# LorenzoNajt/FlipComplexityEmpirical

Measured on AMD Instinct MI355X. Metric: flip proposals/sec (node) 40x40 grid k=2, 1/2/4/8 MI355X; % LDS/HBM roofline, higher is better.
Workload: dtype int8

## Files before the change

flipcomplexityempirical_amd/csrc/fc_capi.cpp:

```cpp
#include <algorithm>
#include <cstdio>
#include <cstdlib>
#include <cstring>
#include <memory>
#include <new>
#include <string>
#include <vector>

#include "fc_run.h"

struct fc_graph {
    fc::HostGraph h;
};

namespace {

constexpr int kWaveSlots = 64;
thread_local std::string g_err;

}

int fc::fail(int code, const std::string &msg) {
    g_err = msg;
    return code;
// ... 228 lines not shown
    for (int32_t c = 0; c < r->n_chains; ++c) {
        fc::ChainScalars &s = sc[c];
        const int64_t w = fc::geom_from(fc::u53(words[2 * c], words[2 * c + 1]), r->log1mp[s.nb]);
        s.sum_wait += w - s.wait_cur;
        s.wait_cur = w;
    }
    HIP_TRY(hipMemcpy(r->d_sc, sc.data(), sc.size() * sizeof(sc[0]), hipMemcpyHostToDevice));
    return FC_OK;
}

#ifdef FC_PHASE_PROF
static int dump_prof(fc_run *r, hipStream_t s) {
    if (const char *path = std::getenv("FC_PROF_OUT")) {
        std::vector<int64_t> h((size_t)r->n_chains * fc::kProfSlots);
        HIP_TRY(hipStreamSynchronize(s));
        HIP_TRY(hipMemcpy(h.data(), r->d_prof, h.size() * 8, hipMemcpyDeviceToHost));
        if (FILE *f = std::fopen(path, "ab")) {
            std::fwrite(h.data(), 8, h.size(), f);
            std::fclose(f);
        }
    }
    return FC_OK;
}
#endif

static fc::KParams flip_params(const fc_run *r, int64_t n_steps, int64_t max_draws) {
    fc::KParams k{};
    k.graph = r->d_graph;
    k.ring_eid = r->d_ring_eid;
    k.n = r->g.n;
    k.n_edges = r->g.n_edges;
    k.n_chains = r->n_chains;
    k.k = r->p.k;
    k.popk = r->d_popk;
    k.all_exact = r->g.n_exact == r->g.n ? 1 : 0;
    k.dgraph = r->dgraph ? 1 : 0;
    k.mcnt = r->d_mcnt;
    k.ngk = r->d_ngk;
    k.wmax = r->wmax > 0 ? r->wmax : 1;
    k.wdyn = r->p.k > 2 && r->wmax <= 0 ? 1 : 0;
    k.nfh = r->d_nfh;
    k.band = r->d_sbits ? 1 : 0;
    k.sbits = r->d_sbits;
    k.band_step0 = 1;
    while (k.band_step0 * 2 < r->words) k.band_step0 *= 2;
    k.chain_lds_bytes = r->chain_lds_bytes;
    k.words = r->words;
    k.lab_words = fc::bfs_lab_words(r->g.n);
    k.lemire_thresh = (uint32_t)((1ull << 32) % (uint64_t)r->g.n);
    k.chain_id_offset = r->p.chain_id_offset;
    k.seed_lo = (uint32_t)r->p.seed;
    k.seed_hi = (uint32_t)(r->p.seed >> 32);
    k.pop_lo = (int32_t)r->p.pop_lo;
    k.n_steps = n_steps;
    k.max_draws = max_draws > 0 ? max_draws : 65536 * std::max<int64_t>(n_steps, 1);
    k.assign = r->d_assign;
    k.fcnt = r->d_fcnt;
    k.sc = r->d_sc;
    k.thresh = r->d_thresh;
    k.log1mp = r->d_log1mp;
    k.pkeys = r->d_pkeys;
    k.labels = r->d_labels;
    k.diag = r->p.diag_mask;
    k.flags = r->p.flags;
    k.cut_hist = r->d_cut_hist;
    k.nb_hist = r->d_nb_hist;
    k.nb_w = r->nb_w;
    k.nb_pairs = (r->p.flags & FC_FLAG_NB_PAIRS) && r->p.k > 2;
    k.edge_acc = r->d_edge_acc;
    k.num_flips = r->d_num_flips;
    k.part_sum = r->d_part_sum;
    k.last_flipped = r->d_last_flipped;
    k.flip_count = r->d_flip_count;
    k.occ_acc = r->d_occ_acc;
    k.last_accept = r->d_last_accept;
    k.trace = r->d_trace;
    k.trace_chains = r->p.trace_chains;
    k.trace_cap = r->p.trace_cap;
    k.tape = r->d_tape;
    k.tape_draws = r->tape_draws;
    k.events = r->d_events;
    k.ev_cap = r->ev_cap;
    k.hit_lo = r->p.hit_lo;
    k.hit_hi = r->p.hit_hi;
    k.nsub = r->tune.nsub;
    k.hit_stop = r->tune.hit_stop;
    k.par_min = r->tune.par_min;
    k.multi_flip = r->tune.multi ? r->mf_marks : 0;
    k.wait_q = r->tune.wait_q;
    k.wpb = r->tune.wpb;
    k.coop = r->tune.coop ? 1 : 0;
    k.variant = r->variant ? 1 : 0;
    k.accept = r->p.accept;
    k.con_valid = r->p.con_valid;
    k.con_accept = r->p.con_accept;
    if (r->variant) k.par_min = kWaveSlots + 1;
    for (int i = 0; i < 3; ++i) {
        k.prio_nb[i] = r->tune.prio_div[0] > 0 && r->p.k == 2 ? k.n / r->tune.prio_div[i] : 0;
        k.prio_th[i] = r->tune.prio_th[i];
    }
    return k;
}

static fc::RecomParams recom_params(const fc_run *r, int64_t n_steps, int64_t max_draws, int64_t *prof) {
    fc::RecomParams q{};
    q.graph = r->d_graph;
    q.nbe = r->d_nbe;
    q.eslot = r->d_eslot;
    q.nb_d = r->nb_d;
    q.eu = r->d_eu;
    q.ev = r->d_ev;
    q.n = r->g.n;
    q.n_edges = r->g.n_edges;
    q.n_chains = r->n_chains;
// ... 91 lines not shown
    HIP_TRY(hipSetDevice(r->p.device));
    fc::KParams k = flip_params(r, n_steps, max_draws);
    hipStream_t s = hip_stream ? (hipStream_t)hip_stream : r->stream;
#ifdef FC_PHASE_PROF
    if (!r->d_prof) {
        if (int rc = r->d_prof.alloc((size_t)r->n_chains * fc::kProfSlots)) return rc;
    }
    HIP_TRY(hipMemsetAsync(r->d_prof, 0, (size_t)r->n_chains * fc::kProfSlots * 8, s));
    k.prof = r->d_prof;
#endif
    size_t slot_i;
    if (int rc = take_event_slot(r, &slot_i)) return rc;
    const auto evp = r->launch_events[slot_i];
    HIP_TRY(hipEventRecord(evp.first, s));
    if (r->p.proposal == FC_PROPOSE_RECOM) {
        const fc::RecomParams q = recom_params(r, n_steps, max_draws, k.prof);
        const int e = fc::launch_recom(q, r->g.ring_max, s, r->kname, sizeof r->kname);
        if (e != 0) return fail(FC_ERR_HIP, std::string("recom kernel launch: ") + hipGetErrorString((hipError_t)e));
        return finish_launches(r, evp, s);
    }
    constexpr int64_t kChunk = int64_t(1) << 24;
    if (r->p.k == 2 && k.prio_nb[0] > 0 && k.prio_th[0] >= 0.0f) {
        if (!r->d_eta) {
            if (int rc = r->d_eta.alloc(2)) return rc;
            HIP_TRY(hipMemsetAsync(r->d_eta, 0, 2 * sizeof(uint32_t), s));
        }
        k.eta = r->d_eta;
    }
    if (r->tune.deal) {
        if (!r->d_deal) {
            if (int rc = r->d_deal.alloc((size_t)fc::kDealKeys + 4)) return rc;
            if (int rc = r->d_order.alloc((size_t)r->n_chains)) return rc;
            if (int rc = r->d_ctime.alloc((size_t)r->n_chains)) return rc;
        }
        k.deal = r->d_deal;
        k.order = r->d_order;
        k.ctime = r->d_ctime;
    }
    int64_t chunk = kChunk;
    if (int rc = size_tally_log(r, n_steps, s, k, &chunk)) return rc;
    for (int64_t done = 0; done < n_steps; done += chunk) {
        k.n_steps = std::min(chunk, n_steps - done);
        if (max_draws <= 0) k.max_draws = 65536 * k.n_steps;
        if (k.order) {
            const int e = fc::launch_deal_order(r->d_ctime, r->d_sc, k.n, r->n_chains, r->deal_timed ? 1 : 0,
                                                r->d_order, r->d_deal, s);
            if (e != 0) return fail(FC_ERR_HIP, std::string("deal kernel launch: ") + hipGetErrorString((hipError_t)e));
            r->deal_timed = true;
        }
        if (k.eta) {
            k.eta_parity = (int32_t)(r->n_flip_launches++ & 1);
            HIP_TRY(hipMemsetAsync(r->d_eta + k.eta_parity, 0, sizeof(uint32_t), s));
        }
        const int e = r->p.k == 2 ? fc::launch_flip2(k, r->g.ring_max, s, r->kname, sizeof r->kname)
                                    : fc::launch_flipk(k, r->g.ring_max, s, r->kname, sizeof r->kname);
        if (e != 0) return fail(FC_ERR_HIP, std::string("flip kernel launch: ") + hipGetErrorString((hipError_t)e));
        if (k.tl_len) {
            const int er = fc::launch_tally_reduce(k, r->g.ring_max, s);
            if (er != 0) return fail(FC_ERR_HIP, std::string("tally reduce launch: ") + hipGetErrorString((hipError_t)er));
        }
    }
    return finish_launches(r, evp, s);
}

int fc_run_sync(fc_run *r) {
    if (!r) return fail(FC_ERR_ARG, "fc_run_sync: null run");
    HIP_TRY(hipSetDevice(r->p.device));
    HIP_TRY(hipDeviceSynchronize());
    return FC_OK;
}

int fc_run_last_ms(fc_run *r, float *ms) {
    if (!r || !ms) return fail(FC_ERR_ARG, "fc_run_last_ms: null argument");
    if (!r->timed) return fail(FC_ERR_ARG, "fc_run_last_ms: no launch recorded");
    HIP_TRY(hipEventSynchronize(r->ev1));
    HIP_TRY(hipEventElapsedTime(ms, r->ev0, r->ev1));
    return FC_OK;
}

int fc_run_timings(fc_run *r, float *ms, int32_t cap, int32_t *n) {
    if (!r || !n || (cap > 0 && !ms)) return fail(FC_ERR_ARG, "fc_run_timings: null argument");
    HIP_TRY(hipSetDevice(r->p.device));
    const size_t cnt = r->n_launch_events, sz = r->launch_events.size();
    if (cnt) HIP_TRY(hipEventSynchronize(r->launch_events[(r->ev_head + cnt - 1) % sz].second));
    int32_t m = 0;
    for (size_t i = 0; i < cnt && m < cap; ++i, ++m) {
        const auto &pr = r->launch_events[(r->ev_head + i) % sz];
        HIP_TRY(hipEventElapsedTime(&ms[m], pr.first, pr.second));
    }
    *n = (int32_t)cnt;
    r->n_launch_events = 0;
    r->ev_head = 0;
    return FC_OK;
}

int fc_host_register(void *ptr, int64_t bytes) {
    if (!ptr || bytes <= 0) return fail(FC_ERR_ARG, "fc_host_register: null or empty buffer");
    HIP_TRY(hipHostRegister(ptr, (size_t)bytes, hipHostRegisterDefault));
    return FC_OK;
}

int fc_host_unregister(void *ptr) {
    if (!ptr) return fail(FC_ERR_ARG, "fc_host_unregister: null buffer");
    HIP_TRY(hipHostUnregister(ptr));
    return FC_OK;
}

// ... 15 lines not shown
```

flipcomplexityempirical_amd/csrc/fc_device.h:

```cpp
#pragma once
#include <hip/hip_runtime.h>
#include <stdint.h>

#include "fc_internal.h"
#include "fc_philox.h"
#include "fc_ring.h"

namespace fc {
namespace dev {

__device__ __forceinline__ void compiler_fence() { asm volatile("" ::: "memory"); }
__device__ __forceinline__ void wave_sync() { asm volatile("s_waitcnt lgkmcnt(0)" ::: "memory"); }

#ifdef FC_PHASE_PROF
#ifdef FC_PHASE_SYNC
#define FC_STAMP(t)                                                    \
    asm volatile("s_waitcnt vmcnt(0) lgkmcnt(0)" ::: "memory");        \
    const int64_t t = (int64_t)__builtin_amdgcn_s_memtime()
#else
#define FC_STAMP(t) const int64_t t = (int64_t)__builtin_amdgcn_s_memtime()
#endif
#define FC_PROF(i, x) \
    do { if (lane == 0) atomicAdd((unsigned long long *)&prof_acc[i], (unsigned long long)(int64_t)(x)); } while (0)
#else
// ... 475 lines not shown
            while (bits) {
                const int b = __builtin_ctzll(bits);
                bits &= bits - 1;
                const NodeRec<RMAX> r = G[i * 64 + b];
                const uint32_t nbr = (uint32_t)(r.meta >> kMetaNbrShift) & 0xffffu;
#pragma unroll
                for (int j = 0; j < RMAX; ++j) {
                    if (!((nbr >> j) & 1u)) continue;
                    const int e = ring_entry<RMAX>(r.ring, j);
                    if (a[e] != A) continue;
                    const uint64_t bit = 1ull << (e & 63);
                    const uint64_t old = atomicOr((unsigned long long *)&S.vis[e >> 6], (unsigned long long)bit);
                    if (!(old & bit)) atomicOr((unsigned long long *)&S.nxt[e >> 6], (unsigned long long)bit);
                }
            }
        }
        wave_sync();
        const bool found = my_target < 0 || ((S.vis[my_target >> 6] >> (my_target & 63)) & 1ull);
        if (__all(found)) return true;
        bool any = false;
        for (int i = lane; i < W; i += kWave) {
            const uint64_t x = S.nxt[i];
            S.front[i] = x;
            S.nxt[i] = 0;
            any |= x != 0;
        }
        wave_sync();
        if (!__any(any)) return false;
    }
}

constexpr uint32_t ST_VS = 1u;
constexpr uint32_t ST_AC = 2u;
constexpr uint32_t ST_IC = 4u;
constexpr uint32_t ST_IP = 8u;
constexpr uint32_t ST_BD = 16u;
constexpr uint32_t ST_BR = 32u;
constexpr uint32_t LF_HIT = 1u << 8;
constexpr uint32_t LF_ACC = 1u << 9;
constexpr uint32_t LF_SLIN = 1u << 10;
constexpr uint32_t LF_SCYC = 1u << 11;
constexpr uint32_t LF_EXACT = 1u << 12;
constexpr uint32_t LF_GAM = 1u << 13;
constexpr uint32_t LF_HAS = 1u << 14;
constexpr uint32_t LF_WROTE = 1u << 15;
constexpr uint32_t LF_FRZ = 1u << 16;

__device__ __attribute__((noinline)) inline int64_t geom_wait_of(uint32_t x0, uint32_t x1, double log1mp) {
    return geom_from(u53(x0, x1), log1mp);
}

}

template <typename P>
inline void launch_lds(void (*kern)(P), dim3 grid, dim3 block, size_t lds, hipStream_t s, const P &p) {
    if (lds > 65536) (void)hipFuncSetAttribute((const void *)kern, hipFuncAttributeMaxDynamicSharedMemorySize, (int)lds);
    hipLaunchKernelGGL(kern, grid, block, lds, s, p);
}

}
```

flipcomplexityempirical_amd/csrc/fc_flip2.hip:

```cpp
#include <hip/hip_runtime.h>

#include <cstdio>
#include <cstdlib>
#include <algorithm>

#include "fc_device.h"
#include "fc_internal.h"
#include "fc_philox.h"
#include "fc_tally.h"

namespace fc {

using namespace dev;

#ifndef FC_PRIO_EVERY_LOG2
#define FC_PRIO_EVERY_LOG2 4
#endif
template <int RMAX, int NSUB, bool FULL, bool SEARCH, bool XTRA, bool BAND>
__global__ __launch_bounds__(256, (RMAX == 8 ? 4 : 1)) void flip2_kernel(KParams p) {
    static_assert(FULL || !XTRA, "XTRA is a FULL instance");
    constexpr int kRV = BAND ? NSUB : 4;
    extern __shared__ __attribute__((aligned(16))) unsigned char smem[];
    const int lane = (int)(threadIdx.x & 63u);
    const int wv = __builtin_amdgcn_readfirstlane((int)(threadIdx.x >> 6));
    const int wave = (int)blockIdx.x * (int)(blockDim.x >> 6) + wv;
    if (wave >= p.n_chains) return;
    const int c = p.order ? deal_chain(p, lane) : wave;

    const int n = p.n;
    const int npad = (n + 15) & ~15;
    unsigned char *base = smem + (size_t)wv * p.chain_lds_bytes;
    int8_t *a = (int8_t *)base;
    uint8_t *fcnt = base + npad;
    uint64_t *T = (uint64_t *)(base + 2 * npad);
    BfsScratch bs{};
    bs.vis = (uint64_t *)(T + (2 * RMAX + 2));
    bs.front = bs.vis + p.words;
    bs.nxt = bs.front + p.words;
    bs.W = p.words;
    bs.prof = nullptr;
    uint32_t *slot = (uint32_t *)(bs.nxt + p.words);
    uint8_t *smark = (uint8_t *)(slot + 5 * 64);
    uint8_t *nmark = smark + npad;
    uint8_t *const dum = nmark + npad + (lane & 15);
#define FC_ST(cond, ref, val) (*((cond) ? (uint8_t *)&(ref) : dum) = (uint8_t)(val))
    uint64_t *q_d = (uint64_t *)(nmark + npad + 16);
    uint32_t *q_nb = (uint32_t *)(q_d + kWaitQ), *q_run = q_nb + kWaitQ;
    uint32_t *q_v = q_run + kWaitQ, *q_c = q_v + kWaitQ;
    uint64_t *misc = (uint64_t *)(q_c + kWaitQ);
    uint64_t *const sb = misc + 5;
    const NodeRec<RMAX> *__restrict__ G = (const NodeRec<RMAX> *)p.graph;

    {
        const uint4 *ga = (const uint4 *)(p.assign + (size_t)c * npad);
        const uint4 *gf = (const uint4 *)(p.fcnt + (size_t)c * npad);
        for (int i = lane; i < npad / 16; i += kWave) {
            ((uint4 *)a)[i] = ga[i];
            ((uint4 *)fcnt)[i] = gf[i];
        }
        if (lane < 2 * RMAX + 1) T[lane] = p.thresh[(size_t)c * (2 * RMAX + 1) + lane];
        for (int i = lane; i < npad / 4 + 2; i += kWave) ((uint64_t *)smark)[i] = ~0ull;
        if (BAND && lane < p.words) sb[lane] = p.sbits[(size_t)c * p.words + lane];
    }
    ChainScalars *scp = p.sc + c;
    uint64_t draw = scp->draw;
    const int64_t steps_in = scp->steps;
    int64_t trace_len = FULL ? scp->trace_len : 0;
    int64_t ev_len = FULL ? scp->ev_len : 0, hit_time = FULL ? scp->hit_time : 0;
    int cut = scp->cut, nb = scp->nb;
    int pops0 = scp->pops[0], pops1 = scp->pops[1];
    const int pop_lo = scp->pop_lo, pop_hi = scp->pop_hi;
    int ng0 = scp->ngamma[0], ng1 = scp->ngamma[1];
    int64_t wait_cur = scp->wait_cur;
    int qn = 0;
    int last_flip = scp->last_flip;
    int stuck = 0;
    int rem = (int)p.n_steps;
    uint64_t draw_cap = draw + (uint64_t)p.max_draws;
    if (XTRA && p.tape && draw_cap > (uint64_t)p.tape_draws) draw_cap = (uint64_t)p.tape_draws;
    const uint32_t chain_gid = p.chain_id_offset + (uint32_t)c;
    const bool force_bfs = (p.flags & FC_FLAG_FORCE_BFS) != 0;
    const bool want_wait = (p.diag & FC_DIAG_WAIT) != 0;
    const bool trace_on = XTRA && p.trace && c < p.trace_chains;
    const bool defer = (want_wait || FULL) && !trace_on && !(XTRA && p.tape);

    int64_t acc_cut = 0, acc_nb = 0, acc_wait = 0, acc_cut2 = 0, acc_nb2 = 0;
    int n_acc = 0, n_ic = 0, n_ip = 0;
    int64_t cnt64 = 0;
    auto cnt_fold = [&]() {
        cnt64 += lane == 0 ? n_acc : lane == 1 ? n_ic : lane == 2 ? n_ip : 0;
        n_acc = n_ic = n_ip = 0;
    };
#ifdef FC_PHASE_PROF
    int64_t *prof_acc = (int64_t *)(base + p.chain_lds_bytes - kProfSlots * 8);
    if (lane < kProfSlots) prof_acc[lane] = 0;
#endif
    wave_sync();
    uint32_t nS = 1u, thrS = 0u;
    auto band_count = [&]() {
        const int cw = lane < p.words ? (int)__popcll(sb[lane]) : 0;
        nS = (uint32_t)rl32(wave_scan_incl(cw), kWave - 1);
        thrS = (0u - nS) % nS;
    };
    auto band_rebuild = [&]() {
        compiler_fence();
        if (lane < p.words) sb[lane] = 0ull;
        compiler_fence();
        for (int j = 0; j < p.words; ++j) {
            const int u = 64 * j + lane;
            const bool isB = u < n && fcnt[u] != 0;
            const uint64_t mb = __ballot(isB);
            if (!mb) continue;
            if (lane == 0) atomicOr((unsigned long long *)&sb[j], (unsigned long long)mb);
            if (isB) {
                const NodeRec<RMAX> ru = G[u];
                const uint32_t nbm = (uint32_t)(ru.meta >> kMetaNbrShift) & 0xffffu;
#pragma unroll
                for (int i = 0; i < RMAX; ++i)
                    if ((nbm >> i) & 1u) {
                        const int w = ring_entry<RMAX>(ru.ring, i);
                        atomicOr((uint32_t *)sb + (w >> 5), 1u << (w & 31));
                    }
            }
        }
        compiler_fence();
        band_count();
    };
    if constexpr (BAND) band_count();
#ifdef FC_PHASE_PROF
    {
        uint32_t hw, xcc;
        asm volatile("s_getreg_b32 %0, hwreg(HW_REG_HW_ID)" : "=s"(hw));
        asm volatile("s_getreg_b32 %0, hwreg(HW_REG_XCC_ID)" : "=s"(xcc));
        FC_PROF(20, (int64_t)(((xcc & 7u) << 12) | ((hw >> 4) & 0xfffu)));
    }
#endif
    FC_STAMP(t_loop0);
// ... 14 lines not shown
                    ev.cut = (uint16_t)(qc & 0x7fffffffu);
                    ev.nb = (uint16_t)nbq;
                    ev.target = (uint8_t)(qc >> 31);
                    ev.reserved = 0;
                    p.events[(size_t)c * p.ev_cap + idx] = ev;
                }
            }
            if (p.diag & (FC_DIAG_HIST | FC_DIAG_FLIPS | FC_DIAG_FLIPS_EXACT | FC_DIAG_EDGES)) {
                const int64_t lbase = (int64_t)misc[3];
                if (p.tl && lbase + qn <= p.tl_cap) {
                    if (in)
                        ((uint4 *)p.tl)[(size_t)c * (size_t)p.tl_cap + (size_t)(lbase + lane)] =
                            tally_pack(t - (int64_t)misc[4], run, qv, qc, (uint32_t)nbq);
                    if (lane == 0) misc[3] = (uint64_t)(lbase + qn);
                } else if (in) {
                    tally_apply<RMAX>(p, c, t, run, qv, qc, (uint32_t)nbq, p.labels[0], p.labels[1]);
                }
            }
            if (p.diag & FC_DIAG_SERIES) ev_len += qn;
        }
    };
    auto wait_flush = [&]() {
        compiler_fence();
        int64_t w = 0;
        if (lane < qn) {
            const uint64_t run = q_run[lane], cq = q_c[lane] & 0x7fffffffu, nq = q_nb[lane];
            const uint64_t cr = cq * run, br = nq * run;
            acc_cut += (int64_t)cr;
            acc_cut2 += (int64_t)(cr * cq);
            acc_nb += (int64_t)br;
            acc_nb2 += (int64_t)(br * nq);
        }
        if (want_wait && lane < qn) {
            const uint64_t dq = q_d[lane];
            const Words4 g = philox4x32_10((uint32_t)dq, (uint32_t)(dq >> 32), chain_gid, 1u, p.seed_lo, p.seed_hi);
            w = geom_wait_of(g.x0, g.x1, p.log1mp[q_nb[lane]]);
            acc_wait += w * (int64_t)q_run[lane];
        }
        tally_flush();
        wait_cur = rl64(w, qn - 1);
        qn = 0;
        compiler_fence();
    };
    int prio = 0;
    if (lane == 0) {
        misc[3] = 0;
        misc[4] = (uint64_t)steps_in;
        if (FULL && p.tl_t0) p.tl_t0[c] = steps_in;
        misc[0] = __builtin_amdgcn_s_memrealtime();
        const float eta0 = p.eta ? (float)p.eta[p.eta_parity ^ 1] * (float)p.n_steps * (1.0f / 1024.0f) : 0.0f;
        misc[1] = (uint64_t)__float_as_uint(eta0);
    }
    compiler_fence();
    const PhiloxKeys pkeys0 = (PhiloxKeys)(uintptr_t)p.pkeys;
    while (rem > 0) {
        const bool every = ((prio += 4) & (((1 << FC_PRIO_EVERY_LOG2) - 1) << 2)) == 0;
        if (every) cnt_fold();
        if (every && p.prio_nb[0] > 0) {
            const int done = (int)p.n_steps - rem;
            const float eta = __uint_as_float((uint32_t)misc[1]);
            int lv;
            if (eta > 0.0f && done * 16 >= (int)p.n_steps) {
                const float pr = (float)(__builtin_amdgcn_s_memrealtime() - misc[0]) * (float)p.n_steps / ((float)done * eta);
                lv = (pr > p.prio_th[0]) + (pr > p.prio_th[1]) + (pr > p.prio_th[2]);
            } else {
                lv = (nb < p.prio_nb[0]) + (nb < p.prio_nb[1]) + (nb < p.prio_nb[2]);
            }
            if (lv != (prio & 3)) {
                prio = (prio & ~3) | lv;
                switch (lv) {
                    case 0: __builtin_amdgcn_s_setprio(0); break;
                    case 1: __builtin_amdgcn_s_setprio(1); break;
                    case 2: __builtin_amdgcn_s_setprio(2); break;
                    default: __builtin_amdgcn_s_setprio(3); break;
                }
            }
        }
        FC_STAMP(t_a);
        FC_PROF(5, 1);
        if (draw >= draw_cap) {
            stuck = 1;
            break;
        }
        const uint64_t room = draw_cap - draw;
        int nh = 0;
        int gen = 0;
        int rv[kRV];
        auto rv_off = [&](int j, int l) { return BAND ? 64 * j + l : 4 * l + j - (int)(draw & 3u); };
        if constexpr (!BAND) {
            const int s0 = (int)(draw & 3u);
            const int wcap = 64 * NSUB < 4 * kWave - s0 ? 64 * NSUB : 4 * kWave - s0;
            const int win = (uint64_t)wcap < room ? wcap : (int)room;
            const uint64_t q = (draw >> 2) + (uint64_t)lane;
            uint32_t nw[4];
            if (XTRA && p.tape) {
#pragma unroll
                for (int j = 0; j < 4; ++j) {
                    const int off = 4 * lane + j - s0;
                    const bool inr = off >= 0 && off < win;
                    nw[j] = p.tape[((size_t)c * (size_t)p.tape_draws + (inr ? draw + (uint64_t)off : draw)) * 6];
                }
            } else {
                PhiloxKeys pk = pkeys0;
                asm volatile("" : "+s"(pk));
                const Words4 w = philox4x32_10_keys((uint32_t)q, (uint32_t)(q >> 32), chain_gid, 3u, pk);
                nw[0] = w.x0;
                nw[1] = w.x1;
                nw[2] = w.x2;
                nw[3] = w.x3;
            }
            int vdj[4];
            uint32_t okm = 0u, hb = 0u;
#pragma unroll
            for (int j = 0; j < 4; ++j) {
                const int off = 4 * lane + j - s0;
                const uint64_t m = (uint64_t)nw[j] * (uint64_t)(uint32_t)n;
                vdj[j] = (int)(m >> 32);
                const bool ok = (off >= 0) & (off < win) & ((uint32_t)m >= p.lemire_thresh);
                okm |= (uint32_t)ok << j;
                hb |= (uint32_t)(ok & (fcnt[vdj[j]] != 0)) << j;
            }
            const int hc = __popc(hb);
            const int incl = wave_scan_incl(hc);
            const int excl = incl - hc;
            const int tot = rl32(incl, kWave - 1);
            gen = win;
            int lim = 4 * kWave;
            if (tot > 64) {
                const int L = __builtin_ctzll(__ballot(incl >= 64));
                const uint32_t hbL = rlu(hb, L);
                const int k = 64 - rl32(excl, L);
                uint32_t mk = hbL;
                for (int i = 1; i < k; ++i) mk &= mk - 1u;
                const int jj = __builtin_ctz(mk);
                lim = 4 * L + jj - s0 + 1;
                gen = lim;
            }
            uint32_t *const ssink = slot + 256 + lane;
#pragma unroll
            for (int j = 0; j < 4; ++j) {
                const int off = 4 * lane + j - s0;
                const int sp = excl + __popc(hb & ((1u << j) - 1u));
                const bool hit = (hb >> j) & 1u;
                const bool put = hit & (sp < 64);
                *(put ? slot + sp : ssink) = (uint32_t)vdj[j];
                *(put ? slot + 192 + sp : ssink) = (uint32_t)off;
                rv[j] = (((okm >> j) & 1u) & !hit & (off < lim)) ? (vdj[j] | (sp << 16)) : -1;
            }
            nh = tot;
        } else {
            int bpre = 0x7fffffff;
            {
                const int cw = lane < p.words ? (int)__popcll(sb[lane]) : 0;
                const int inc = wave_scan_incl(cw);
                if (lane < p.words) bpre = inc - cw;
            }
#pragma unroll
// ... 8 lines not shown
                const int idx = (int)(m >> 32);
                const bool okd = inrange && (uint32_t)m >= thrS;
                int bw = 0, bb = 0;
                for (int st2 = p.band_step0; st2 >= 1; st2 >>= 1) {
                    const int cand = bw + st2;
                    const int pc = __builtin_amdgcn_ds_bpermute(cand << 2, bpre);
                    if (pc <= idx) {
                        bw = cand;
                        bb = pc;
                    }
                }
                const int vd = 64 * bw + select_bit64(sb[bw], idx - bb);
                const bool hitd = okd & (fcnt[vd] != 0);
                const uint64_t hm = __ballot(hitd);
                const int sp = nh + count_below(hm);
                if (hitd && sp < 64) {
                    slot[sp] = (uint32_t)vd;
                    slot[64 + sp] = w.x1;
                    slot[128 + sp] = w.x2;
                    slot[192 + sp] = (uint32_t)off;
                }
                const int cnt = __popcll(hm);
                int used = kWave;
                if (nh + cnt > 64) {
                    used = kth_set_bit(hm, 64 - nh) + 1;
                    gen += used;
                } else {
                    gen = (uint64_t)(gen + 64) < room ? gen + 64 : (int)room;
                }
                rv[r] = (okd & !hitd & (lane < used)) ? (vd | (sp << 16)) : rv[r];
                nh += cnt;
            }
        }
        const int ns = nh < 64 ? nh : 64;
        compiler_fence();
        FC_STAMP(t_b);
        FC_PROF(1, t_b - t_a);

        const bool has = lane < ns;
        const int off_r = (int)slot[192 + lane], v_r = (int)slot[lane];
        int off_l = has ? off_r : gen;
        const uint64_t d = draw + (uint64_t)off_l;
        int v = has ? v_r : 0;
        uint32_t w1, w2;
        if constexpr (BAND) {
            w1 = slot[64 + lane];
            w2 = slot[128 + lane];
        } else {
            if (XTRA && p.tape) {
                const uint32_t *t = p.tape + ((size_t)c * (size_t)p.tape_draws + (has ? d : draw)) * 6;
                w1 = t[1];
                w2 = t[2];
            } else {
                PhiloxKeys pk = pkeys0;
                asm volatile("" : "+s"(pk));
                const Words4 g = philox4x32_10_keys((uint32_t)d, (uint32_t)(d >> 32), chain_gid, 0u, pk);
                w1 = g.x1;
                w2 = g.x2;
            }
            slot[64 + lane] = w1;
            slot[128 + lane] = w2;
        }
        const NodeRec<RMAX> rec = G[v];
        int av = a[v];
        int pv = rec.pop;
        const uint32_t Ln = (uint32_t)(rec.meta & kMetaLenMask);
        const uint32_t full = (1u << Ln) - 1u;
        uint32_t nbr = (uint32_t)(rec.meta >> kMetaNbrShift) & 0xffffu;
        const uint32_t link = (uint32_t)(rec.meta >> kMetaLinkShift) & 0xffffu;
        int cell[RMAX];
        uint32_t in1 = 0;
        int ad[RMAX];
#pragma unroll
        for (int i = 0; i < RMAX; ++i) {
            cell[i] = ring_entry<RMAX>(rec.ring, i);
            ad[i] = a[cell[i]];
        }
#pragma unroll
        for (int i = 0; i < RMAX; ++i) asm volatile("" : "+v"(ad[i]));
#pragma unroll
        for (int i = 0; i < RMAX; ++i) in1 |= (uint32_t)ad[i] << i;
        uint32_t inA = (av ? in1 : ~in1) & full;
        slot[256 + lane] = link | (Ln << 16);
        const uint32_t nbrA = inA & nbr;
        uint32_t tmask = nbr & ~inA;
        int nA = __popc(nbrA);
        int delta = nA - __popc(tmask);
        const bool hit = has && tmask != 0u;
        bool s_lin, s_cyc;
        {
            const uint32_t rot = Ln ? (((inA >> 1) | (inA << (Ln - 1))) & full) : 0u;
            const uint32_t lk = inA & rot & link;
            s_lin = one_run_flat(nbrA, full & ~lk, full);
            const uint32_t vlink = (Ln >= 2) ? ((inA & (inA >> (Ln - 1)) & 1u) << (Ln - 1)) : 0u;
            s_cyc = one_run_flat(nbrA, full & ~(lk | vlink), full);
        }
        const bool exact = SEARCH ? (rec.meta & kMetaExact) && !force_bfs : true;
        const bool gam = (rec.meta & kMetaGamma) != 0;
        const bool acc = mant53(w1, w2) < T[delta + RMAX];
        uint32_t st = (hit ? LF_HIT : 0u) | (acc ? LF_ACC : 0u) | (s_lin ? LF_SLIN : 0u) | (s_cyc ? LF_SCYC : 0u) |
                      (exact ? LF_EXACT : 0u) | (gam ? LF_GAM : 0u) | (has ? LF_HAS : 0u);
        if (XTRA && (rec.meta & kMetaFrozen)) st |= LF_FRZ;
#ifdef FC_PHASE_PROF
        bool first_it = true;
#endif
        FC_STAMP(t_c);
        FC_PROF(2, t_c - t_b);

        int end = ns, pos = 0;
        int trunc_off = gen;
        bool target_hit = false;
        bool rebuild = false;
        const int cut0 = cut, nb0 = nb;
        const int64_t steps0 = FULL ? steps_in + ((int)p.n_steps - rem) : 0;
        const int last_flip0 = last_flip;
        const int a_last0 = FULL && last_flip0 >= 0 ? (int)a[last_flip0] : 0;
        int cut_after = 0, nb_after = 0;
        auto dp_of = [&]() { return av == 0 ? -pv : pv; };
        auto dg_of = [&]() { return (st & LF_GAM) ? (av == 0 ? -1 : 1) : 0; };

        auto reeval = [&](int from, int vfx, uint32_t eqx) {
            FC_STAMP(t_re0);
            compiler_fence();
            if (has && lane >= from) {
                const uint32_t lkl = slot[256 + lane];
                const uint32_t w1r = slot[64 + lane], w2r = slot[128 + lane];
                if (vfx < 0) {
                    av = a[v];
                    uint32_t i1 = 0;
                    int ad[RMAX];
#pragma unroll
                    for (int i = 0; i < RMAX; ++i) ad[i] = a[cell[i]];
#pragma unroll
                    for (int i = 0; i < RMAX; ++i) asm volatile("" : "+v"(ad[i]));
#pragma unroll
                    for (int i = 0; i < RMAX; ++i) i1 |= (uint32_t)ad[i] << i;
                    inA = av ? i1 : ~i1;
                } else {
                    const bool self = v == vfx;
                    av = self ? 1 - av : av;
                    inA = (self ? ~inA : inA) ^ eqx;
                }
                const uint32_t nbA = inA & nbr;
                tmask = nbr & ~inA;
                nA = __popc(nbA);
                delta = nA - __popc(tmask);
                const uint64_t th = T[delta + RMAX];
                const uint32_t lnk = lkl & 0xffffu, L2 = lkl >> 16;
                const uint32_t fl = (1u << L2) - 1u;
                inA &= fl;
                const uint32_t rot = L2 ? (((inA >> 1) | (inA << (L2 - 1))) & fl) : 0u;
                const uint32_t lk = inA & rot & lnk;
                const bool sl = one_run_flat(nbA, fl & ~lk, fl);
                const uint32_t vlink = (L2 >= 2) ? ((inA & (inA >> (L2 - 1)) & 1u) << (L2 - 1)) : 0u;
                const bool sc = one_run_flat(nbA, fl & ~(lk | vlink), fl);
                const bool ac = mant53(w1r, w2r) < th;
                st = (st & (LF_EXACT | LF_GAM | LF_HAS | LF_FRZ)) | (tmask != 0u ? LF_HIT : 0u) | (ac ? LF_ACC : 0u) |
                     (sl ? LF_SLIN : 0u) | (sc ? LF_SCYC : 0u);
            }
            compiler_fence();
            FC_STAMP(t_re1);
            FC_PROF(16, t_re1 - t_re0);
            FC_PROF(17, 1);
        };

        auto run_bfs = [&](int f) -> bool {
            const uint32_t nbrAf = rlu(inA & nbr, f);
            int my_target = -1, start = -1;
#pragma unroll
            for (int k2 = 0; k2 < RMAX / 2; ++k2) {
                const uint32_t wrd = rlu(rec.ring[k2], f);
                if ((lane >> 1) == k2) my_target = (int)((wrd >> (16 * (lane & 1))) & 0xffffu);
                if (start < 0 && ((nbrAf >> (2 * k2)) & 1u)) start = (int)(wrd & 0xffffu);
                if (start < 0 && ((nbrAf >> (2 * k2 + 1)) & 1u)) start = (int)(wrd >> 16);
            }
            if (!(lane < RMAX && ((nbrAf >> lane) & 1u))) my_target = -1;
            int64_t lv = 0;
            const bool res = wave_bfs_single<RMAX>(G, a, bs, lane, rl32(v, f), rl32(av, f), my_target, start, lv);
            if (lane == 0) {
// ... 548 lines not shown
        const uint64_t el = __builtin_amdgcn_s_memrealtime() - misc[0];
        atomicMax(&p.eta[p.eta_parity], (uint32_t)min(el * 1024ull / (uint64_t)max((int)p.n_steps, 1), 0xffffffffull));
    }
#ifdef FC_PHASE_PROF
    wave_sync();
    if (p.prof && lane == 0)
        for (int i = 0; i < kProfSlots; ++i) p.prof[(size_t)c * kProfSlots + i] = prof_acc[i];
#endif

    {
        uint4 *ga = (uint4 *)(p.assign + (size_t)c * npad);
        uint4 *gf = (uint4 *)(p.fcnt + (size_t)c * npad);
        for (int i = lane; i < npad / 16; i += kWave) {
            ga[i] = ((const uint4 *)a)[i];
            gf[i] = ((const uint4 *)fcnt)[i];
        }
        if (BAND && lane < p.words) p.sbits[(size_t)c * p.words + lane] = sb[lane];
    }
    cnt_fold();
    const int taken = (int)p.n_steps - rem;
    const int64_t cnt_acc = rl64(cnt64, 0), cnt_ic = rl64(cnt64, 1), cnt_ip = rl64(cnt64, 2);
    const int64_t cnt_prop = (int64_t)taken + cnt_ic + cnt_ip;
    wave_sum64_all(acc_cut, acc_nb, acc_wait, acc_cut2, acc_nb2);
    if (FULL && p.tl_len && lane == 0) p.tl_len[c] = (int64_t)misc[3];
    if (lane == 0) {
        scp->draw = draw;
        scp->steps = steps_in + taken;
        scp->proposals += cnt_prop;
        scp->accepted += cnt_acc;
        scp->inv_contig += cnt_ic;
        scp->inv_pop += cnt_ip;
        if (FULL) {
            scp->trace_len = trace_len;
            scp->ev_len = ev_len;
            scp->hit_time = hit_time;
        }
        scp->sum_cut += acc_cut;
        scp->sum_nb += acc_nb;
        scp->sum_wait += acc_wait;
        scp->sum_cut2 += acc_cut2;
        scp->sum_nb2 += acc_nb2;
        scp->cut = cut;
        scp->nb = nb;
        scp->pops[0] = pops0;
        scp->pops[1] = pops1;
        scp->ngamma[0] = ng0;
        scp->ngamma[1] = ng1;
        scp->wait_cur = wait_cur;
        scp->last_flip = last_flip;
        scp->stuck = stuck;
    }
}

int launch_flip2(const KParams &p, int ring_max, void *stream, char *name, size_t name_cap) {
    const int wpb = p.wpb;
    const int blocks = (p.n_chains + wpb - 1) / wpb;
    const size_t lds = (size_t)p.chain_lds_bytes * wpb;
    hipStream_t s = (hipStream_t)stream;
    const dim3 grid(blocks), block(kWave * wpb);
    const bool full = p.tape || p.trace || (p.diag & ~(uint32_t)FC_DIAG_WAIT) || p.hit_lo <= p.hit_hi || p.variant;
    const bool xtra = p.tape || p.trace || p.variant;
    const bool search = !p.all_exact || (p.flags & FC_FLAG_FORCE_BFS);
#define FC_LAUNCH2B(R, S, F, X, Y, B)                                                                      \
    do {                                                                                                    \
        if (name)                                                                                           \
            snprintf(name, name_cap, "fc::flip2_kernel<%d, %d, %s, %s, %s, %s>", R, S, F ? "true" : "false", \
                     X ? "true" : "false", Y ? "true" : "false", B ? "true" : "false");                    \
        launch_lds(flip2_kernel<R, S, F, X, Y, B>, grid, block, lds, s, p);                                 \
    } while (0)
#define FC_LAUNCH2(R, S, F, X, Y)                        \
    do {                                                 \
        if (p.band) FC_LAUNCH2B(R, S, F, X, Y, true);    \
        else FC_LAUNCH2B(R, S, F, X, Y, false);          \
    } while (0)
#define FC_SEARCH2(R, S, F, Y)                    \
    do {                                          \
        if (search) FC_LAUNCH2(R, S, F, true, Y);  \
        else FC_LAUNCH2(R, S, F, false, Y);        \
    } while (0)
#define FC_FULL2(R, S)                                \
    do {                                              \
        if (xtra) FC_SEARCH2(R, S, true, true);        \
        else if (full) FC_SEARCH2(R, S, true, false);  \
        else FC_SEARCH2(R, S, false, false);           \
    } while (0)
#define FC_NSUB2(R)                                \
    switch (p.nsub) {                              \
        case 1: FC_FULL2(R, 1); break;             \
        case 2: FC_FULL2(R, 2); break;             \
        case 4: FC_FULL2(R, 4); break;             \
        default: return (int)hipErrorInvalidValue; \
    }
    if (ring_max == 8) {
        FC_NSUB2(8)
    } else if (ring_max == 16) {
        FC_NSUB2(16)
    } else {
        return (int)hipErrorInvalidValue;
    }
#undef FC_NSUB2
#undef FC_FULL2
#undef FC_SEARCH2
#undef FC_LAUNCH2
#undef FC_LAUNCH2B
    return (int)hipGetLastError();
}

}
```

flipcomplexityempirical_amd/csrc/fc_internal.h:

```cpp
#pragma once

#include <stddef.h>
#include <stdint.h>

#include <string>
#include <vector>

#include "../../include/flipchain.h"
#include "fc_replay.h"

namespace fc {

constexpr int kWave = 64;
constexpr int kWavesPerBlock = 4;
constexpr int kBigChainLds = 16 * 1024;
inline int bfs_lab_words(int n) { return ((n + 3) / 4 + 1) & ~1; }
inline int bfs_bytes(int n) { return 4 * bfs_lab_words(n) + 128 + 16 + 2 * 2 * 512 + 24 * ((n + 63) / 64); }
inline int waves_per_block(int chain_lds_bytes) { return chain_lds_bytes > kBigChainLds ? 1 : kWavesPerBlock; }
constexpr int kMaxK = 2;
constexpr int kMaxKGeneral = 32;
constexpr int kMaxKDistrictRule = 31;
inline int dgraph_lds_bytes(int k) { return 4 * k * k + 4 * 32 + 4 * 32; }
constexpr int hb_bytes(int ring_max) { return ring_max == 8 ? 256 : 128; }

// ... 8 lines not shown
struct alignas(16) NodeRec {
    uint64_t meta;
    int32_t pop;
    int32_t deg;
    uint32_t ring[RMAX / 2];
};
static_assert(sizeof(NodeRec<8>) == 32, "NodeRec<8> must be 32 B");
static_assert(sizeof(NodeRec<16>) == 48, "NodeRec<16> must be 48 B");

struct HostGraph {
    int32_t n = 0, n_edges = 0, ring_max = 8, max_degree = 0;
    std::vector<int32_t> row_ptr, col_idx, pop;
    std::vector<double> pos;
    std::vector<int32_t> eu, ev;
    std::vector<int32_t> ring;
    std::vector<uint64_t> meta;
    std::vector<int32_t> ring_eid;
    int32_t n_exact = 0, n_gamma = 0;
    bool planar = false, outer_simple = false, connected = false;
};

std::string build_host_graph(int32_t n, const int32_t *row_ptr, const int32_t *col_idx,
                             const int32_t *pop, const double *pos_xy, uint32_t flags, HostGraph &g);

struct ChainScalars {
    uint64_t draw;
    int64_t steps, proposals, accepted, inv_contig, inv_pop;
    int64_t sum_cut, sum_nb, sum_wait, sum_cut2, sum_nb2;
    int64_t wait_cur;
    int64_t bfs_calls, bfs_levels;
    int64_t trace_len;
    int64_t ev_len;
    int64_t hit_time;
    int64_t ser_t0;
    int32_t cut, nb;
    int32_t pops[kMaxK];
    int32_t ngamma[kMaxK];
    int32_t last_flip;
    int32_t stuck;
    int32_t ser_cut0, ser_nb0;
    int32_t pop_lo, pop_hi;
};

struct KParams {
    const void *graph;
    const int32_t *ring_eid;
    int32_t n, n_edges, n_chains, k;
    int32_t chain_lds_bytes;
    int32_t words;
    int32_t lab_words;
    uint32_t lemire_thresh;
    uint32_t chain_id_offset;
    uint32_t seed_lo, seed_hi;
    int32_t pop_lo;
    const uint32_t *pkeys;
    int64_t n_steps;
    int64_t max_draws;
    int8_t *assign;
    uint8_t *fcnt;
    ChainScalars *sc;
    const uint64_t *thresh;
    const double *log1mp;
    const int32_t *labels;
    uint32_t diag;
    uint32_t flags;
    int64_t *cut_hist;
    int64_t *nb_hist;
    int32_t nb_w;
    int32_t nb_pairs;
    int64_t *edge_acc;
    int64_t *num_flips;
    int64_t *part_sum;
    int64_t *last_flipped;
    int64_t *flip_count;
    int64_t *occ_acc;
    int64_t *last_accept;
    fc_record *trace;
    int32_t trace_chains;
    int64_t trace_cap;
    const uint32_t *tape;
    int64_t tape_draws;
    int32_t *popk;
    int32_t wmax;
    int32_t wdyn;
    int32_t *nfh;
    fc_event *events;
    int64_t ev_cap;
    int32_t hit_lo, hit_hi;
    int32_t nsub;
    int32_t hit_stop;
    int64_t *prof;
    int32_t par_min;
    int32_t variant;
    int32_t accept;
    uint32_t con_valid;
    uint32_t con_accept;
    int32_t prio_nb[3];
    uint32_t *eta;
    int32_t eta_parity;
    float prio_th[3];
    int32_t wait_q;
    int32_t wpb;
    int32_t all_exact;
    int32_t dgraph;
    int32_t *mcnt;
    int32_t *ngk;
    int32_t coop;
    uint32_t *deal;
    const uint32_t *order;
    uint32_t *ctime;
    int32_t multi_flip;
    uint32_t *tl;
    int64_t *tl_t0;
    int64_t *tl_len;
    int64_t tl_cap;
    int32_t band;
    int32_t band_step0;
    uint64_t *sbits;
};
static_assert(offsetof(KParams, pkeys) == 64 && offsetof(KParams, n_steps) == 72, "KParams: pkeys fills pop_hi's slot");

constexpr int kDealKeys = 1 << 15;

constexpr int kProfSlots = 32;
constexpr int kWaitQ = 64;
constexpr int kWaitQK = 32;
constexpr int kNfh = 32;

struct RecomParams {
    const void *graph;
    const uint32_t *nbe;
    const uint32_t *eslot;
    const int32_t *eu, *ev;
    int32_t nb_d;
    int32_t n, n_edges, n_chains, chain_lds_bytes;
    uint32_t chain_id_offset, seed_lo, seed_hi;
    int32_t pop_lo, pop_hi;
    double pop_target, epsilon;
    int32_t node_repeats, max_attempts;
    int64_t n_steps, max_draws;
    int8_t *assign;
    ChainScalars *sc;
    const uint64_t *accept_thresh;
    fc_recom_record *trace;
    int32_t trace_chains;
    int64_t trace_cap;
    int64_t *prof;
};
inline int recom_lds_bytes(int n, int ring_max) { return (ring_max == 8 ? 14 : 15) * ((n + 15) & ~15); }
int launch_recom(const RecomParams &p, int ring_max, void *stream, char *name, size_t name_cap);

int launch_flipk(const KParams &p, int ring_max, void *stream, char *name, size_t name_cap);
int launch_flip2(const KParams &p, int ring_max, void *stream, char *name, size_t name_cap);
int launch_tally_reduce(const KParams &p, int ring_max, void *stream);
int launch_deal_order(const uint32_t *ctime, const ChainScalars *sc, int n, int n_chains, int timed,
                      uint32_t *order, uint32_t *deal, void *stream);

int launch_series_expand(const fc_event *events, int64_t ev_cap, const int64_t *ev_len, const int64_t *t0,
                         const int32_t *cut0, const int64_t *len, int32_t c0, int32_t nc, int64_t stride,
                         int64_t max_len, uint16_t *x, void *stream);
int launch_series_lagsums(const uint16_t *x, const int64_t *len, int32_t c0, int32_t nc, int64_t stride,
                          int64_t max_len, const int32_t *lags, int32_t nlags, unsigned long long *sums,
                          void *stream);

constexpr int kFrameWaves = 4;
enum FrameMode { kFrameEvents = 0, kFrameCount = 1, kFrameWrite = 2, kFrameStage = 3 };
struct FrameParams {
    LogWindow log;
    int32_t n_frame;
    const int32_t *fu, *fv;
    const double *mid;
    double cx, cy;
    const int32_t *tog_idx;
    const uint64_t *tog_mask;
    int32_t n_rows;
    int64_t cap;
    double *slope, *angle;
    int32_t *n_cut;
    int64_t *t_out;
    int64_t *cp_cnt;
    const int64_t *cp_off;
    int64_t *wcnt;
};
int launch_frame(const FrameParams &p, int mode, void *stream);
int launch_frame_compact(int32_t nc, int64_t stage_cap, const int64_t *st_t, const double *st_s,
                         const double *st_a, const int64_t *wcnt, const int64_t *cp_off, int64_t *t_out,
                         double *slope, double *angle, void *stream);

}
```

flipcomplexityempirical_amd/csrc/fc_philox.h:

```cpp
#pragma once
#include <stdint.h>

#include <cmath>

#if defined(__HIPCC__) || defined(__HIP__)
#define FC_HD __host__ __device__ __forceinline__
#else
#define FC_HD inline
#endif

namespace fc {

struct Words4 {
    uint32_t x0, x1, x2, x3;
};

FC_HD Words4 philox4x32_10(uint32_t c0, uint32_t c1, uint32_t c2, uint32_t c3, uint32_t k0, uint32_t k1) {
#pragma unroll
    for (int r = 0; r < 10; ++r) {
        if (r) {
            k0 += 0x9E3779B9u;
            k1 += 0xBB67AE85u;
#if defined(__HIP_DEVICE_COMPILE__)
            asm volatile("" : "+s"(k0), "+s"(k1));
#endif
        }
        const uint64_t p0 = (uint64_t)0xD2511F53u * c0, p1 = (uint64_t)0xCD9E8D57u * c2;
#if defined(__HIP_DEVICE_COMPILE__)
        const uint32_t n0 = __builtin_amdgcn_bitop3_b32((uint32_t)(p1 >> 32), c1, k0, 0x96);
        const uint32_t n2 = __builtin_amdgcn_bitop3_b32((uint32_t)(p0 >> 32), c3, k1, 0x96);
#else
        const uint32_t n0 = (uint32_t)(p1 >> 32) ^ c1 ^ k0, n2 = (uint32_t)(p0 >> 32) ^ c3 ^ k1;
#endif
        c0 = n0;
        c1 = (uint32_t)p1;
        c2 = n2;
        c3 = (uint32_t)p0;
    }
    return Words4{c0, c1, c2, c3};
}

constexpr int kPhiloxKeyWords = 20;
inline void philox_round_keys(uint32_t k0, uint32_t k1, uint32_t *out) {
    for (int r = 0; r < 10; ++r) {
        out[2 * r] = k0 + (uint32_t)r * 0x9E3779B9u;
        out[2 * r + 1] = k1 + (uint32_t)r * 0xBB67AE85u;
    }
}
#if defined(__HIPCC__) || defined(__HIP__)
typedef const uint32_t __attribute__((address_space(4))) *PhiloxKeys;
__device__ __forceinline__ Words4 philox4x32_10_keys(uint32_t c0, uint32_t c1, uint32_t c2, uint32_t c3, PhiloxKeys kp) {
    uint32_t K[kPhiloxKeyWords];
#pragma unroll
    for (int i = 0; i < kPhiloxKeyWords; ++i) K[i] = kp[i];
#pragma unroll
    for (int r = 0; r < 10; ++r) {
        const uint64_t p0 = (uint64_t)0xD2511F53u * c0, p1 = (uint64_t)0xCD9E8D57u * c2;
#if defined(__HIP_DEVICE_COMPILE__)
        const uint32_t n0 = __builtin_amdgcn_bitop3_b32((uint32_t)(p1 >> 32), c1, K[2 * r], 0x96);
        const uint32_t n2 = __builtin_amdgcn_bitop3_b32((uint32_t)(p0 >> 32), c3, K[2 * r + 1], 0x96);
#else
        const uint32_t n0 = (uint32_t)(p1 >> 32) ^ c1 ^ K[2 * r], n2 = (uint32_t)(p0 >> 32) ^ c3 ^ K[2 * r + 1];
#endif
        c0 = n0;
        c1 = (uint32_t)p1;
        c2 = n2;
        c3 = (uint32_t)p0;
    }
    return Words4{c0, c1, c2, c3};
}
#endif

FC_HD uint64_t mant53(uint32_t a, uint32_t b) { return ((uint64_t)(a >> 5) << 26) | (uint64_t)(b >> 6); }

FC_HD double u53(uint32_t a, uint32_t b) { return (double)mant53(a, b) * (1.0 / 9007199254740992.0); }

constexpr double kWaitCap = 4611686018427387904.0;
FC_HD int64_t geom_from(double U, double log1mp) {
    const double q = log(1.0 - U) / log1mp;
    if (!(fabs(q) < kWaitCap)) return (int64_t)kWaitCap;
    return (int64_t)ceil(q) - 1;
}

}
```

Baseline: 21.04 billion.

## Pass Philox key pointer as separate kernel arg and keep draws in registers

```diff
diff --git a/flipcomplexityempirical_amd/csrc/fc_capi.cpp b/flipcomplexityempirical_amd/csrc/fc_capi.cpp
--- a/flipcomplexityempirical_amd/csrc/fc_capi.cpp
+++ b/flipcomplexityempirical_amd/csrc/fc_capi.cpp
@@ -304,6 +304,7 @@
     k.seed_lo = (uint32_t)r->p.seed;
     k.seed_hi = (uint32_t)(r->p.seed >> 32);
     k.pop_lo = (int32_t)r->p.pop_lo;
+    k.pop_hi = (int32_t)r->p.pop_hi;
     k.n_steps = n_steps;
     k.max_draws = max_draws > 0 ? max_draws : 65536 * std::max<int64_t>(n_steps, 1);
     k.assign = r->d_assign;
@@ -311,7 +312,6 @@
     k.sc = r->d_sc;
     k.thresh = r->d_thresh;
     k.log1mp = r->d_log1mp;
-    k.pkeys = r->d_pkeys;
     k.labels = r->d_labels;
     k.diag = r->p.diag_mask;
     k.flags = r->p.flags;
@@ -509,7 +509,7 @@
             k.eta_parity = (int32_t)(r->n_flip_launches++ & 1);
             HIP_TRY(hipMemsetAsync(r->d_eta + k.eta_parity, 0, sizeof(uint32_t), s));
         }
-        const int e = r->p.k == 2 ? fc::launch_flip2(k, r->g.ring_max, s, r->kname, sizeof r->kname)
+        const int e = r->p.k == 2 ? fc::launch_flip2(k, r->d_pkeys, r->g.ring_max, s, r->kname, sizeof r->kname)
                                     : fc::launch_flipk(k, r->g.ring_max, s, r->kname, sizeof r->kname);
         if (e != 0) return fail(FC_ERR_HIP, std::string("flip kernel launch: ") + hipGetErrorString((hipError_t)e));
         if (k.tl_len) {
diff --git a/flipcomplexityempirical_amd/csrc/fc_device.h b/flipcomplexityempirical_amd/csrc/fc_device.h
--- a/flipcomplexityempirical_amd/csrc/fc_device.h
+++ b/flipcomplexityempirical_amd/csrc/fc_device.h
@@ -551,10 +551,10 @@
 
 }
 
-template <typename P>
-inline void launch_lds(void (*kern)(P), dim3 grid, dim3 block, size_t lds, hipStream_t s, const P &p) {
+template <typename... P>
+inline void launch_lds(void (*kern)(P...), dim3 grid, dim3 block, size_t lds, hipStream_t s, const P &...p) {
     if (lds > 65536) (void)hipFuncSetAttribute((const void *)kern, hipFuncAttributeMaxDynamicSharedMemorySize, (int)lds);
-    hipLaunchKernelGGL(kern, grid, block, lds, s, p);
-}
-
-}
+    hipLaunchKernelGGL(kern, grid, block, lds, s, p...);
+}
+
+}
diff --git a/flipcomplexityempirical_amd/csrc/fc_flip2.hip b/flipcomplexityempirical_amd/csrc/fc_flip2.hip
--- a/flipcomplexityempirical_amd/csrc/fc_flip2.hip
+++ b/flipcomplexityempirical_amd/csrc/fc_flip2.hip
@@ -16,8 +16,22 @@
 #ifndef FC_PRIO_EVERY_LOG2
 #define FC_PRIO_EVERY_LOG2 4
 #endif
+static_assert(sizeof(KParams) % 8 == 0, "flip2_kernel's second argument sits at sizeof(KParams)");
+template <bool FULL>
+__device__ __forceinline__ PhiloxKeys batch_keys(PhiloxKeys keys) {
+    typedef const unsigned char __attribute__((address_space(4))) *KernArg;
+    if constexpr (FULL) {
+        KernArg ka = (KernArg)__builtin_amdgcn_kernarg_segment_ptr();
+        asm volatile("" : "+s"(ka));
+        return *(const PhiloxKeys __attribute__((address_space(4))) *)(ka + sizeof(KParams));
+    } else {
+        asm volatile("" : "+s"(keys));
+        return keys;
+    }
+}
+
 template <int RMAX, int NSUB, bool FULL, bool SEARCH, bool XTRA, bool BAND>
-__global__ __launch_bounds__(256, (RMAX == 8 ? 4 : 1)) void flip2_kernel(KParams p) {
+__global__ __launch_bounds__(256, (RMAX == 8 ? 4 : 1)) void flip2_kernel(KParams p, PhiloxKeys keys) {
     static_assert(FULL || !XTRA, "XTRA is a FULL instance");
     constexpr int kRV = BAND ? NSUB : 4;
     extern __shared__ __attribute__((aligned(16))) unsigned char smem[];
@@ -82,7 +96,7 @@
     const bool force_bfs = (p.flags & FC_FLAG_FORCE_BFS) != 0;
     const bool want_wait = (p.diag & FC_DIAG_WAIT) != 0;
     const bool trace_on = XTRA && p.trace && c < p.trace_chains;
-    const bool defer = (want_wait || FULL) && !trace_on && !(XTRA && p.tape);
+    const bool defer = (!FULL && !BAND) || ((want_wait || FULL) && !trace_on && !(XTRA && p.tape));
 
     int64_t acc_cut = 0, acc_nb = 0, acc_wait = 0, acc_cut2 = 0, acc_nb2 = 0;
     int n_acc = 0, n_ic = 0, n_ip = 0;
@@ -203,7 +217,6 @@
         misc[1] = (uint64_t)__float_as_uint(eta0);
     }
     compiler_fence();
-    const PhiloxKeys pkeys0 = (PhiloxKeys)(uintptr_t)p.pkeys;
     while (rem > 0) {
         const bool every = ((prio += 4) & (((1 << FC_PRIO_EVERY_LOG2) - 1) << 2)) == 0;
         if (every) cnt_fold();
@@ -252,8 +265,7 @@
                     nw[j] = p.tape[((size_t)c * (size_t)p.tape_draws + (inr ? draw + (uint64_t)off : draw)) * 6];
                 }
             } else {
-                PhiloxKeys pk = pkeys0;
-                asm volatile("" : "+s"(pk));
+                const PhiloxKeys pk = batch_keys<FULL>(keys);
                 const Words4 w = philox4x32_10_keys((uint32_t)q, (uint32_t)(q >> 32), chain_gid, 3u, pk);
                 nw[0] = w.x0;
                 nw[1] = w.x1;
@@ -368,14 +380,15 @@
                 w1 = t[1];
                 w2 = t[2];
             } else {
-                PhiloxKeys pk = pkeys0;
-                asm volatile("" : "+s"(pk));
+                const PhiloxKeys pk = batch_keys<FULL>(keys);
                 const Words4 g = philox4x32_10_keys((uint32_t)d, (uint32_t)(d >> 32), chain_gid, 0u, pk);
                 w1 = g.x1;
                 w2 = g.x2;
             }
-            slot[64 + lane] = w1;
-            slot[128 + lane] = w2;
+            if constexpr (FULL) {
+                slot[64 + lane] = w1;
+                slot[128 + lane] = w2;
+            }
         }
         const NodeRec<RMAX> rec = G[v];
         int av = a[v];
@@ -440,7 +453,7 @@
             compiler_fence();
             if (has && lane >= from) {
                 const uint32_t lkl = slot[256 + lane];
-                const uint32_t w1r = slot[64 + lane], w2r = slot[128 + lane];
+                const uint32_t w1r = (!FULL && !BAND) ? w1 : slot[64 + lane], w2r = (!FULL && !BAND) ? w2 : slot[128 + lane];
                 if (vfx < 0) {
                     av = a[v];
                     uint32_t i1 = 0;
@@ -1095,12 +1108,13 @@
     }
 }
 
-int launch_flip2(const KParams &p, int ring_max, void *stream, char *name, size_t name_cap) {
+int launch_flip2(const KParams &p, const uint32_t *pkeys, int ring_max, void *stream, char *name, size_t name_cap) {
     const int wpb = p.wpb;
     const int blocks = (p.n_chains + wpb - 1) / wpb;
     const size_t lds = (size_t)p.chain_lds_bytes * wpb;
     hipStream_t s = (hipStream_t)stream;
     const dim3 grid(blocks), block(kWave * wpb);
+    const PhiloxKeys keys = (PhiloxKeys)(uintptr_t)pkeys;
     const bool full = p.tape || p.trace || (p.diag & ~(uint32_t)FC_DIAG_WAIT) || p.hit_lo <= p.hit_hi || p.variant;
     const bool xtra = p.tape || p.trace || p.variant;
     const bool search = !p.all_exact || (p.flags & FC_FLAG_FORCE_BFS);
@@ -1109,7 +1123,7 @@
         if (name)                                                                                           \
             snprintf(name, name_cap, "fc::flip2_kernel<%d, %d, %s, %s, %s, %s>", R, S, F ? "true" : "false", \
                      X ? "true" : "false", Y ? "true" : "false", B ? "true" : "false");                    \
-        launch_lds(flip2_kernel<R, S, F, X, Y, B>, grid, block, lds, s, p);                                 \
+        launch_lds(flip2_kernel<R, S, F, X, Y, B>, grid, block, lds, s, p, keys);                           \
     } while (0)
 #define FC_LAUNCH2(R, S, F, X, Y)                        \
     do {                                                 \
diff --git a/flipcomplexityempirical_amd/csrc/fc_internal.h b/flipcomplexityempirical_amd/csrc/fc_internal.h
--- a/flipcomplexityempirical_amd/csrc/fc_internal.h
+++ b/flipcomplexityempirical_amd/csrc/fc_internal.h
@@ -84,8 +84,7 @@
     uint32_t lemire_thresh;
     uint32_t chain_id_offset;
     uint32_t seed_lo, seed_hi;
-    int32_t pop_lo;
-    const uint32_t *pkeys;
+    int32_t pop_lo, pop_hi;
     int64_t n_steps;
     int64_t max_draws;
     int8_t *assign;
@@ -150,7 +149,6 @@
     int32_t band_step0;
     uint64_t *sbits;
 };
-static_assert(offsetof(KParams, pkeys) == 64 && offsetof(KParams, n_steps) == 72, "KParams: pkeys fills pop_hi's slot");
 
 constexpr int kDealKeys = 1 << 15;
 
@@ -183,7 +181,7 @@
 int launch_recom(const RecomParams &p, int ring_max, void *stream, char *name, size_t name_cap);
 
 int launch_flipk(const KParams &p, int ring_max, void *stream, char *name, size_t name_cap);
-int launch_flip2(const KParams &p, int ring_max, void *stream, char *name, size_t name_cap);
+int launch_flip2(const KParams &p, const uint32_t *pkeys, int ring_max, void *stream, char *name, size_t name_cap);
 int launch_tally_reduce(const KParams &p, int ring_max, void *stream);
 int launch_deal_order(const uint32_t *ctime, const ChainScalars *sc, int n, int n_chains, int timed,
                       uint32_t *order, uint32_t *deal, void *stream);
diff --git a/flipcomplexityempirical_amd/csrc/fc_philox.h b/flipcomplexityempirical_amd/csrc/fc_philox.h
--- a/flipcomplexityempirical_amd/csrc/fc_philox.h
+++ b/flipcomplexityempirical_amd/csrc/fc_philox.h
@@ -49,7 +49,9 @@
 }
 #if defined(__HIPCC__) || defined(__HIP__)
 typedef const uint32_t __attribute__((address_space(4))) *PhiloxKeys;
-__device__ __forceinline__ Words4 philox4x32_10_keys(uint32_t c0, uint32_t c1, uint32_t c2, uint32_t c3, PhiloxKeys kp) {
+#endif
+template <typename KP>
+FC_HD Words4 philox4x32_10_keys(uint32_t c0, uint32_t c1, uint32_t c2, uint32_t c3, KP kp) {
     uint32_t K[kPhiloxKeyWords];
 #pragma unroll
     for (int i = 0; i < kPhiloxKeyWords; ++i) K[i] = kp[i];
@@ -69,7 +71,6 @@
     }
     return Words4{c0, c1, c2, c3};
 }
-#endif
 
 FC_HD uint64_t mant53(uint32_t a, uint32_t b) { return ((uint64_t)(a >> 5) << 26) | (uint64_t)(b >> 6); }
 
```

After: 21.51 billion, median of 6. +2.2%, better.
